# lawfuyang/HobbyRenderer

Measured on AMD Instinct MI355X. Metric: Mrays/s at 1920×1080, 8 spp, 4 bounces; 1/2/4/8 GPU scaling, higher is better.
Workload: dtype f32; 1 GPU; config 2: Cornell-box-class procedural scene (38 triangles, 9 instances, closed room, emissive quad + default sun), 1920x1080, 8 spp (accumulation indices 0..7), 4 bounces; frames_in_flight=2, serial_kernels=False, mode=default

## Files before the change

hobbyrenderer_amd/csrc/pt_capi.cpp:

```cpp
#include <hip/hip_runtime.h>

#include <chrono>
#include <cmath>
#include <cstdio>
#include <cstdlib>
#include <cstring>
#include <mutex>
#include <new>
#include <stdexcept>
#include <limits>
#include <string>
#include <system_error>
#include <thread>
#include <vector>

#include "../../include/hobbyrt_pt.h"
#include "bvh_build.h"
#include "bvh_build_gpu.h"
#include "pt_deform.h"
#include "pt_skin.h"
#include "pt_anim.h"
#include "pt_device.h"
#include "pt_kernels.h"
#include "pt_motion.h"
// ... 188 lines not shown
    if (const char* e = getenv("HRPT_WF_SEGMENT_SHIFT")) c->wf.knobs.segmentShift = (uint32_t)atoi(e);
    if (const char* e = getenv("HRPT_WF_SEGMENT_SIZE")) c->wf.knobs.segmentSize = (uint32_t)atoi(e);
    if (const char* e = getenv("HRPT_WF_BLOCKS_PER_CU")) c->wf.knobs.blocksPerCu = (uint32_t)atoi(e);
    if (const char* e = getenv("HRPT_WF_EXTEND_BLOCKS_PER_CU")) c->wf.knobs.extendBlocksPerCu = (uint32_t)atoi(e);
    if (const char* e = getenv("HRPT_WF_REFILL_MIN")) c->wf.knobs.refillMin = (uint32_t)atoi(e);
    if (const char* e = getenv("HRPT_WF_BVH_WIDTH")) c->wf.knobs.bvhWidth = (uint32_t)atoi(e);
    if (const char* e = getenv("HRPT_BVH_BUILDER")) c->bvhBuilder = (strcmp(e, "ploc") == 0 || strcmp(e, "2") == 0) ? HRPT_BVH_BUILDER_GPU_PLOC : ((strcmp(e, "gpu") == 0 || strcmp(e, "lbvh") == 0 || strcmp(e, "1") == 0) ? HRPT_BVH_BUILDER_GPU_LBVH : ((strcmp(e, "auto") == 0 || strcmp(e, "3") == 0) ? HRPT_BVH_BUILDER_AUTO : HRPT_BVH_BUILDER_HOST_SAH));
    if (const char* e = getenv("HRPT_WF_PAD_LDS")) c->wf.knobs.padLdsBytes = (uint32_t)atoi(e);
    if (const char* e = getenv("HRPT_WF_DRAIN_SEGMENTS")) c->wf.knobs.drainSegments = atoi(e) != 0;
    if (const char* e = getenv("HRPT_WF_SERIAL_SHADOW")) c->wf.knobs.serialShadow = atoi(e) != 0;
    if (const char* e = getenv("HRPT_WF_SHADOW_PATH")) c->wf.knobs.shadowPath = atoi(e);
    if (const char* e = getenv("HRPT_WF_SHADE_SORT")) c->wf.knobs.shadeSort = atoi(e) != 0 ? 1 : 0;
    if (const char* e = getenv("HRPT_WF_SLIM_SHADOW")) c->wf.knobs.noSlimShadow = atoi(e) == 0;
    if (const char* e = getenv("HRPT_WF_FUSED_PRIMARY")) c->wf.knobs.noFusedPrimary = atoi(e) == 0;
    if (const char* e = getenv("HRPT_WF_FUSED_BOUNCE0")) c->wf.knobs.noFusedBounce0 = atoi(e) == 0;
    if (const char* e = getenv("HRPT_WF_SHADE_LDS_TABLES")) c->wf.knobs.noShadeLdsTables = atoi(e) == 0;
    if (const char* e = getenv("HRPT_WF_NODE_LOOP_MIN")) c->wf.knobs.nodeLoopMin = (uint32_t)atoi(e);
    if (const char* e = getenv("HRPT_BLOOM_FUSED_TAIL")) { const int v = atoi(e); c->bloomTailTexels = v == 1 ? 8192u : (v > 0 ? (uint32_t)v : 0u); }
    *out = c;
    return HRPT_OK;
}

void hrpt_destroy(HrptContext* c)
{
    if (!c) return;
    (void)hipSetDevice(c->device);
    if (c->stream) (void)hipStreamSynchronize(c->stream);
    free_scene(c);
    for (AnimDeviceCopy& a : c->animations) free_animation_copy(a);
    wavefront_release(c->wf);
// ... 1873 lines not shown
```

hobbyrenderer_amd/csrc/pt_device.h:

```cpp
#pragma once

#include <hip/hip_runtime.h>
#include <stdint.h>

#include "../../include/hobbyrt_pt.h"
#include "../../include/hobbyrt/detmath.h"
#include "../../include/hobbyrt/srgb_table.h"

#define HRT_DEV __device__ __forceinline__

#if defined(HRPT_PHASE_PROFILE) && defined(HRPT_PHASE_TU)
extern __device__ unsigned long long g_phaseCounters[128];
#define HRT_PHASE(k)                                                                                                      \
    do {                                                                                                                  \
        const unsigned long long m_ = __ballot(true);                                                                     \
        if ((threadIdx.x & 63u) == (unsigned)(__ffsll((long long)m_) - 1)) {                                              \
            atomicAdd(&g_phaseCounters[2 * (k)], 1ull); atomicAdd(&g_phaseCounters[2 * (k) + 1], (unsigned long long)__popcll(m_)); \
        }                                                                                                                 \
    } while (0)
#else
#define HRT_PHASE(k) do { } while (0)
#endif
enum {
    PH_EXT_ITER = 0, PH_EXT_REFILL, PH_EXT_NODE, PH_EXT_LEAF, PH_EXT_TRI, PH_EXT_FINISH, PH_EXT_CANDIDATE,
    PH_ANY_ITER = 8, PH_ANY_REFILL, PH_ANY_NODE, PH_ANY_LEAF, PH_ANY_TRI, PH_ANY_FINISH,
    PH_SHADE_ITER = 16, PH_SHADE_HIT, PH_SHADE_ATTR, PH_SHADE_TEX, PH_SHADE_TRANS, PH_SHADE_NEE, PH_SHADE_LOBE_BEGIN, PH_SHADE_DIFFUSE, PH_SHADE_SPEC,
    PH_SHADE_SKY, PH_SHADE_WRITE, PH_SHADE_SORT,
    PH_SHADOW_ENTRY = 32, PH_SHADOW_SAMPLE, PH_SHADOW_QUERY, PH_SHADOW_CONTRIB, PH_SHADOW_RAYS_ITEM,
    PH_COUNT = 40
};

namespace hrt {

struct f2 { float x, y; };
struct f3 { float x, y, z; };
struct f4 { float x, y, z, w; };

HRT_DEV f3 mk3(float x, float y, float z) { f3 r; r.x = x; r.y = y; r.z = z; return r; }
HRT_DEV f3 mk3(const float* p) { return mk3(p[0], p[1], p[2]); }
HRT_DEV f3 operator+(f3 a, f3 b) { return mk3(a.x + b.x, a.y + b.y, a.z + b.z); }
HRT_DEV f3 operator-(f3 a, f3 b) { return mk3(a.x - b.x, a.y - b.y, a.z - b.z); }
HRT_DEV f3 operator*(f3 a, f3 b) { return mk3(a.x * b.x, a.y * b.y, a.z * b.z); }
HRT_DEV f3 operator*(f3 a, float s) { return mk3(a.x * s, a.y * s, a.z * s); }
HRT_DEV f3 operator/(f3 a, float s) { return mk3(a.x / s, a.y / s, a.z / s); }
// ... 306 lines not shown
                    best.t = take ? t : best.t; best.u = take ? u : best.u; best.v = take ? v : best.v;
                    best.inst = take ? inst : best.inst; best.prim = take ? prim : best.prim; best.tri = take ? first + i : best.tri;
                    best.opaque = take ? (__float_as_uint(c.w) & 1u) : best.opaque;
                    best.valid = best.valid || take;
                    tlim = take ? t : tlim;
                }
            }
            if (sp == 0) break;
            cur = stack.pop(--sp);
        }
    }
    return best;
}

template <class BVH, class STACK>
HRT_DEV bool any_opaque(const BVH& bvh, int32_t rootLeaf, uint32_t nodeCount, const Ray& r, STACK& stack, bool& sawNonOpaque, uint32_t nodeLoopMin = 0)
{
    sawNonOpaque = false;
    if (!(r.d.x == r.d.x && r.d.y == r.d.y && r.d.z == r.d.z)) return false;
    RayShear sh = make_shear(r.d);
    f3 inv = traversal_rcp(r.d), noi = slab_origin_term(r.o, inv);
    int sp = 0; int32_t cur;
    if (nodeCount == 0) { if (rootLeaf == 0) return false; cur = rootLeaf; }
    else cur = 0;
    for (;;) {
        while (cur >= 0) {
            cur = inner_step(bvh, cur, noi, inv, r.tmin, r.tmax, stack, sp);
            if ((uint32_t)__popcll(__ballot(cur >= 0)) < nodeLoopMin) break;
        }
        if (cur == kTraversalDone) break;
        if (cur < 0) {
            uint32_t enc = (uint32_t)(~cur);
            uint32_t first = enc >> 2, count = (enc & 3u) + 1u;
            for (uint32_t i = 0; i < count; ++i) {
                float4 a, b, c; bvh.tri(first + i, a, b, c);
                float t, u, v;
                if (tri_test(mk3(a.x, a.y, a.z), mk3(b.x, b.y, b.z), mk3(c.x, c.y, c.z), r, sh, t, u, v)) {
                    if (__float_as_uint(c.w) & 1u) return true;
                    sawNonOpaque = true;
                }
            }
            if (sp == 0) break;
            cur = stack.pop(--sp);
        }
    }
    return false;
}

constexpr int32_t kExitBlas = 0x7FFFFFFE;
struct GlobalBvhTl : GlobalBvh4 {
    static constexpr bool kTwoLevel = true;
    const GpuInstance* instances;
};
struct TlCull { f3 inv, noi, noiF; int32_t inst; };
HRT_DEV void tl_world(TlCull& c, const Ray& r)
{
    c.inv = traversal_rcp(r.d); c.noi = slab_origin_term(r.o, c.inv); c.noiF = c.noi; c.inst = -1;
}
HRT_DEV void tl_enter(TlCull& c, const GpuInstance& I, int32_t inst, const Ray& r)
// ... 733 lines not shown
```

hobbyrenderer_amd/csrc/pt_path.h:

```cpp
#pragma once

#include "pt_device.h"

namespace hrt {

struct PathState {
    Ray ray;
    uint32_t rng;
    f3 throughput, radiance;
    bool inVolume; float interiorIOR; f3 sigmaA, sigmaS;
};

struct SurfaceCarry {
    f3 N, V, worldPos, baseColor, F0; float Fr, roughness, metallic, ior;
    uint32_t rngBeforeLights;
    uint32_t material;
};

HRT_DEV void init_path(PathState& ps, const HrptPathTracerConstants& cb, uint32_t px, uint32_t py)
{
    float u = (((float)px + 0.5f) + cb.m_Jitter[0]) * cb.m_View.m_ViewportSizeInv[0];
    float v = (((float)py + 0.5f) + cb.m_Jitter[1]) * cb.m_View.m_ViewportSizeInv[1];
    float cx = u * 2.0f + -1.0f, cy = v * -2.0f + 1.0f;
    const float* M = cb.m_View.m_MatClipToWorldNoOffset;
// ... 283 lines not shown
    }
    if (overflow) {
        float4 la, lb, lc; bvh.tri(lastTri, la, lb, lc);
        HitKey lower; lower.have = true; lower.t = lastT; lower.inst = __float_as_uint(la.w); lower.prim = __float_as_uint(lb.w);
        for (;;) {
            Hit h = closest_any(bvh, s.rootLeaf, s.nodeCount, ray, lower, stack);
            if (!h.valid) break;
            if (h.opaque) return 0.0f;
            if (shadow_candidate(s, ray, h.t, h.tri, h.u, h.v, st)) return 0.0f;
            lower.t = h.t; lower.inst = h.inst; lower.prim = h.prim;
        }
    }
    return shadow_finish(ray, st);
}
template <int K, class BVH, class STACK, class CAND>
HRT_DEV float shadow_query_buffered(const SceneView& s, const BVH& bvh, f3 worldPos, f3 L, float maxDist, STACK& stack, CAND& cand, uint32_t nodeLoopMin = 0)
{
    Ray ray = shadow_ray(worldPos, L, maxDist);
    if (!(ray.d.x == ray.d.x && ray.d.y == ray.d.y && ray.d.z == ray.d.z)) return 1.0f;
    RayShear sh = make_shear(ray.d);
    f3 inv = traversal_rcp(ray.d), noi = slab_origin_term(ray.o, inv);
    int sp = 0, count = 0; bool overflow = false;
    int32_t cur;
    if (s.nodeCount == 0) { if (s.rootLeaf == 0) return 1.0f; cur = s.rootLeaf; } else cur = 0;
    for (;;) {
        while (cur >= 0) {
            cur = inner_step(bvh, cur, noi, inv, ray.tmin, ray.tmax, stack, sp);
            if ((uint32_t)__popcll(__ballot(cur >= 0)) < nodeLoopMin) break;
        }
        if (cur == kTraversalDone) break;
        if (cur >= 0) continue;
        uint32_t enc = (uint32_t)(~cur);
        uint32_t first = enc >> 2, n = (enc & 3u) + 1u;
        for (uint32_t i = 0; i < n; ++i) {
            float4 a, b, c; bvh.tri(first + i, a, b, c);
            float t, u, v;
            if (!tri_test(mk3(a.x, a.y, a.z), mk3(b.x, b.y, b.z), mk3(c.x, c.y, c.z), ray, sh, t, u, v)) continue;
            if (__float_as_uint(c.w) & 1u) return 0.0f;
            candidate_insert<K>(bvh, cand, count, overflow, t, first + i, __float_as_uint(a.w), __float_as_uint(b.w));
        }
        if (sp == 0) break;
        cur = stack.pop(--sp);
    }
    return shadow_resolve_candidates(s, bvh, ray, sh, count, overflow, cand, stack);
}

template <bool DIRONLY>
HRT_DEV bool nee_draw(const HrptGPULight& l, f3 N, f3 worldPos, f3 sunDirection, uint32_t& rng, float& ux, float& uy)
{
    if (DIRONLY || l.m_Type == HRPT_LIGHT_DIRECTIONAL) {
        if (dot(N, sunDirection) <= 0.0f) return false;
    } else if (!DIRONLY && (l.m_Type == HRPT_LIGHT_POINT || l.m_Type == HRPT_LIGHT_SPOT)) {
        if (l.m_Intensity <= 0.0f) return false;
// ... 228 lines not shown
```

hobbyrenderer_amd/csrc/pt_wavefront.hip:

```cpp
#define HRPT_PHASE_TU 1
#include "pt_wavefront.h"

#include <mutex>
#include <type_traits>
#include <unordered_map>
#include <vector>

#include "bvh_build.h"
#include "pt_gbuffer.h"
#include "pt_motion.h"
#include "pt_path.h"

#ifdef HRPT_PHASE_PROFILE
__device__ unsigned long long g_phaseCounters[128];
#endif
#ifdef HRPT_SKY_DEBUG
__device__ float g_skyDebug[2048 * 16];
#endif

namespace hrt {

namespace {

constexpr uint32_t kMaxSppPerBatch = 64;
// ... 1013 lines not shown
                if (!valid) a.b.shVis[id] = kVisNoRay;
            }
            const unsigned long long m = __ballot(valid);
            if (valid) {
                const uint32_t o = segBase * a.maxLights + outCount + prefix_rank(m);
                a.b.sqO[o] = make_float4(ray.o.x, ray.o.y, ray.o.z, ray.tmin);
                a.b.sqD[o] = make_float4(ray.d.x, ray.d.y, ray.d.z, ray.tmax);
                a.b.sqId[o] = id;
            }
            outCount += (uint32_t)__popcll(m);
        }
        if (lane == 0) a.b.sqCnt[seg] = outCount;
    }
}

template <bool LDS_BVH, int DEPTH, int W, bool DIRONLY, int MODE, int TL = 0>
__global__ __launch_bounds__(kBlock) __attribute__((amdgpu_waves_per_eu(MODE == 2 && TL == 0 ? 4 : ((MODE == 1 || TL != 0) ? 3 : 1)))) void wf_shadow(WfArgs a, HrptPathTracerConstants cb, int bounce)
{
    static_assert(!TL || (!LDS_BVH && W == 4 && (MODE == kShadowOpaque || MODE == kShadowSlim)), "two-level structure: opaque any-hit query over the global tree");
    static_assert(W != kQuantisedTree || (!LDS_BVH && !TL), "quantised nodes: flat tree in global memory");
    constexpr bool NONOPAQUE = MODE == kShadowBuffered || MODE == kShadowResolve;
    constexpr bool SLIM = MODE == kShadowSlim;
    constexpr int kLdsMax = MODE == kShadowResolve ? kExtendLdsStack : kShadowLdsStack;
    extern __shared__ __attribute__((aligned(128))) char smem[];
    LdsStack<DEPTH, kLdsMax> stack; LdsBvh<W> lbvh;
    constexpr size_t candBytes = MODE == kShadowBuffered ? (size_t)kShadowCandidates * 2 * kBlock * 4 : 0;
    setup_lds<LDS_BVH, DEPTH, W>(smem, a.scene, stack, lbvh, candBytes);
    if (DEPTH > kLdsMax) { stack.spill = a.spill[1] + blockIdx.x * kBlock + threadIdx.x; stack.spillStride = gridDim.x * kBlock; }
    LdsCandidates cand; cand.base = reinterpret_cast<int32_t*>(smem + (size_t)LdsStack<DEPTH, kLdsMax>::kRows * kBlock * 4) + threadIdx.x;
    LdsCandidates3 cand3; cand3.base = cand.base;
    typename GlobalBvhOf<(TL ? kTwoLevelTree : W)>::type gbvh = GlobalBvhOf<(TL ? kTwoLevelTree : W)>::make(a.scene);
    const SceneView& s = a.scene;
    const f3 sunDir = mk3(cb.m_SunDirection[0], cb.m_SunDirection[1], cb.m_SunDirection[2]);
    const float sunIntensity = s.lights[0].m_Intensity;

    const uint32_t wavesPerBlock = kBlock / 64, lane = lane_id();
    const uint32_t gw = uniform(blockIdx.x * wavesPerBlock + (threadIdx.x >> 6)), totalWaves = gridDim.x * wavesPerBlock;
    unsigned int nRays = 0, nSamples = 0, nRadiance = 0, nSkipped16 = 0;
    auto process = [&](uint32_t e) {
                HRT_PHASE(PH_SHADOW_ENTRY);
                if (SLIM) {
                    const float4 h0 = a.b.sh0[e], h1 = a.b.sh1[e];
                    const uint32_t slot = __float_as_uint(h0.w);
                    const float4 rd = a.b.rayD[a.shadowParity][slot];
                    const f3 origin = mk3(h0.x, h0.y, h0.z), N = mk3(h1.x, h1.y, h1.z);
                    uint32_t rng = __float_as_uint(rd.w);
                    const float ux = hrt_rng_next(&rng), uy = hrt_rng_next(&rng);
                    ++nSamples;
                    HrptGPULight l = load_light(s, 0u);
                    f3 L; float maxDist;
                    if (!nee_direction<true>(l, N, origin, sunDir, cb.m_CosSunAngularRadius, ux, uy, L, maxDist)) return;
                    float shadow;
                    if (LDS_BVH) shadow = shadow_query<true>(s, lbvh, origin, L, maxDist, stack);
// ... 40 lines not shown
                    if (MODE == kShadowResolve || j) ls = a.b.shL[(size_t)e * a.maxLights + j];
                    HrptGPULight l = load_light(s, __float_as_uint(ls.z));
                    f3 L; float maxDist;
                    if (!nee_direction<DIRONLY>(l, N, origin, sunDir, cb.m_CosSunAngularRadius, ls.x, ls.y, L, maxDist)) continue;
                    float shadow;
                    HRT_PHASE(PH_SHADOW_QUERY);
                    if (MODE == kShadowResolve) {
                        if (vis == kVisClear) shadow = 1.0f;
                        else {
                            Ray sr = shadow_ray(origin, L, maxDist);
                            GlobalCandidates gc; gc.base = a.b.sqCand + (size_t)(e * a.maxLights + j) * kShadowCandidates;
                            const int cnt = (int)((vis >> 8) & 0xFFu); const bool ovf = (vis >> 16) & 1u;
                            if (LDS_BVH) shadow = shadow_resolve_candidates(s, lbvh, sr, make_shear(sr.d), cnt, ovf, gc, stack);
                            else shadow = shadow_resolve_candidates(s, gbvh, sr, make_shear(sr.d), cnt, ovf, gc, stack);
                        }
                    } else if (MODE == kShadowBuffered) {
                        if (LDS_BVH) shadow = shadow_query_buffered<kShadowCandidates>(s, lbvh, origin, L, maxDist, stack, cand);
                        else shadow = shadow_query_buffered<kShadowCandidates>(s, gbvh, origin, L, maxDist, stack, cand);
                    } else {
                        if (LDS_BVH) shadow = shadow_query<true>(s, lbvh, origin, L, maxDist, stack);
                        else if constexpr (TL == 2) shadow = shadow_query_two_level_buffered<kTwoLevelCandidates>(s, gbvh, shadow_ray(origin, L, maxDist), stack, cand3);
                    else shadow = shadow_query<true>(s, gbvh, origin, L, maxDist, stack);
                    }
                    ++nRays;
                    if (shadow != 0.0f) {
                        HRT_PHASE(PH_SHADOW_CONTRIB);
                        float4 h2 = a.b.sh2[e], h3 = a.b.sh3[e];
                        f3 dif, spec;
                        nee_contribution<DIRONLY>(s, l, nee_lighting(N, mk3(h2.x, h2.y, h2.z), mk3(h3.x, h3.y, h3.z), h1.w, h2.w, h3.w), origin, sunDir,
                                                  sunIntensity, L, dif, spec);
                        totalDiffuse = totalDiffuse + dif * shadow;
                        if (bounce == 0) totalSpecular = totalSpecular + spec * shadow;
                    }
                }
                f3 dsum = totalDiffuse + (bounce == 0 ? totalSpecular : mk3(0.0f, 0.0f, 0.0f));
                if (dsum.x != 0.0f || dsum.y != 0.0f || dsum.z != 0.0f) {
                    f3 term = T * dsum;
                    float4 r = a.b.radiance[smp];
                    r.x = r.x + term.x; r.y = r.y + term.y; r.z = r.z + term.z;
                    a.b.radiance[smp] = r;
                    ++nRadiance;
                }
    };
    if (NONOPAQUE) {
        uint32_t seg = gw, cnt = 0, segBase = 0, next = 0; bool haveSeg = false;
        auto open_segment = [&]() {
            haveSeg = false; cnt = 0; next = 0;
            for (; seg < a.numSegments; seg += totalWaves) {
                cnt = uniform(a.b.shadowCnt[seg]);
                if (cnt) { segBase = seg * a.segSize; haveSeg = true; break; }
            }
        };
        open_segment();
        while (haveSeg) {
            uint32_t e = 0xFFFFFFFFu, filled = 0;
            while (filled < 64u && haveSeg) {
                uint32_t take = cnt - next < 64u - filled ? cnt - next : 64u - filled;
                if (lane >= filled && lane < filled + take) e = segBase + next + (lane - filled);
                next += take; filled += take;
// ... 4 lines not shown
    } else {
        for (uint32_t seg = gw; seg < a.numSegments; seg += totalWaves) {
            const uint32_t cnt = uniform(a.b.shadowCnt[seg]), segBase = seg * a.segSize;
            for (uint32_t base = 0; base < cnt; base += 64) {
                uint32_t i = base + lane;
                if (i < cnt) process(segBase + i);
            }
        }
    }
    block_count_add(&a.counters->closestRays, 1, nRays);
    __syncthreads();
    block_count_add(&a.counters->closestRays, 4, nSamples);
    __syncthreads();
    block_count_add(&a.counters->closestRays, 6, nRadiance);
    if (SLIM && a.primary) { __syncthreads(); block_count_add(&a.counters->closestRays, 7, nSkipped16); }
}

__global__ __launch_bounds__(kBlock) void wf_resolve(WfArgs a, float4* __restrict__ accumulation, float4* __restrict__ output, uint32_t firstIndex)
{
    uint32_t p = blockIdx.x * blockDim.x + threadIdx.x;
    uint32_t stride = gridDim.x * blockDim.x;
    for (; p < a.pixelsPadded; p += stride) {
        uint32_t tile = p >> 6, within = p & 63u;
        uint32_t tcol, trow; tile_position(a, tile, tcol, trow);
        uint32_t px = a.rect.column_x(tcol) + (within & 7u), py = a.rect.y0 + trow * 8u + (within >> 3);
        if (px >= a.rect.x1 || py >= a.rect.y1) continue;
        size_t idx = (size_t)py * a.imageWidth + px;
        float4 acc = make_float4(0.0f, 0.0f, 0.0f, 0.0f);
        for (uint32_t k = 0; k < a.spp; ++k) {
            float4 r = a.b.radiance[(size_t)k * a.pixelsPadded + p];
// ... 115 lines not shown

void launch_extend(const Variant& v, uint32_t cus, dim3 g, hipStream_t st, const WfArgs& a, uint32_t parity, bool anyHit = false)
{
    dispatch_variant(v, [&](auto L, auto D, auto W, auto TL) {
        constexpr bool l = L(); constexpr int d = D(), w = W(), tl = TL();
        auto closest = [&](auto kernel) { launch_rounds(cus, kernel, g, v.ldsBytes, st, a, parity); };
        if constexpr (tl != 0) {
            if (a.primary) closest(wf_extend<false, d, 4, false, tl, true>);
            else closest(wf_extend<false, d, 4, false, tl, false>);
        } else if (anyHit) hipLaunchKernelGGL((wf_extend<l, d, w, true>), g, dim3(kBlock), v.ldsBytes + kCandidateLdsBytes, st, a, parity);
        else if constexpr (w == 2) closest(wf_extend<l, d, w, false>);
        else if (a.primary) { if (a.allOpaque) closest(wf_extend<l, d, w, false, 0, true, true>); else closest(wf_extend<l, d, w, false, 0, true>); }
        else { if (a.allOpaque) closest(wf_extend<l, d, w, false, 0, false, true>); else closest(wf_extend<l, d, w, false>); }
    });
}
void launch_shadow(const Variant& v, dim3 g, hipStream_t st, const WfArgs& a, const HrptPathTracerConstants& cb, int bounce, bool dirOnly, int mode)
{
    dispatch_variant(v, [&](auto L, auto D, auto W, auto TL) {
        constexpr bool l = L(); constexpr int d = D(), w = W(), tl = TL();
        auto launch = [&](auto kernel, size_t extraLds) { hipLaunchKernelGGL(kernel, g, dim3(kBlock), v.ldsBytes + extraLds, st, a, cb, bounce); };
        if constexpr (tl != 0) {
            const size_t cand = tl == 2 ? (size_t)kTwoLevelCandidates * 3 * kBlock * 4 : 0;
            if (mode == kShadowSlim) launch(wf_shadow<false, d, 4, true, kShadowSlim, tl>, cand);
            else if (dirOnly) launch(wf_shadow<false, d, 4, true, kShadowOpaque, tl>, cand);
            else launch(wf_shadow<false, d, 4, false, kShadowOpaque, tl>, cand);
        } else if (mode == kShadowResolve) launch(wf_shadow<l, d, w, false, kShadowResolve>, 0);
        else if (mode == kShadowBuffered) launch(wf_shadow<l, d, w, false, kShadowBuffered>, kCandidateLdsBytes);
        else if (mode == kShadowSlim) launch(wf_shadow<l, d, w, true, kShadowSlim>, 0);
        else if (dirOnly) launch(wf_shadow<l, d, w, true, kShadowOpaque>, 0);
        else launch(wf_shadow<l, d, w, false, kShadowOpaque>, 0);
    });
}
void launch_wf_trace_rays(const Variant& v, uint32_t cus, dim3 g, hipStream_t st, const WfTraceArgs& a, bool shadow)
{
    dispatch_variant(v, [&](auto L, auto D, auto W, auto TL) {
        constexpr bool l = L(), tl = TL() != 0; constexpr int d = D(), w = W();
        if constexpr (w != 2) {
            if (shadow) launch_rounds(cus, wf_trace_rays<l, d, w, true, tl>, g, v.ldsBytes + (tl ? 0 : kCandidateLdsBytes), st, a);
            else launch_rounds(cus, wf_trace_rays<l, d, w, false, tl>, g, v.ldsBytes, st, a);
        }
    });
// ... 254 lines not shown
            if (!st.auxStream && hipStreamCreateWithFlags(&st.auxStream, hipStreamNonBlocking) != hipSuccess) { st.auxStream = nullptr; overlap = false; }
            while (overlap && st.forkEvents.size() < (size_t)maxBounces) {
                hipEvent_t f, j;
                if (hipEventCreateWithFlags(&f, hipEventDisableTiming) != hipSuccess) { overlap = false; break; }
                if (hipEventCreateWithFlags(&j, hipEventDisableTiming) != hipSuccess) { (void)hipEventDestroy(f); overlap = false; break; }
                st.forkEvents.push_back(f); st.joinEvents.push_back(j);
            }
        }
        auto shadow_stage = [&](hipStream_t sst, int bounce) {
            a.shadowParity = (uint32_t)bounce & 1u;
            if (plan.shadowMode == kShadowResolve) {
                if (traits.directionalLightsOnly) hipLaunchKernelGGL((wf_shadow_rays<true>), grid, dim3(kBlock), 0, sst, a, cb);
                else hipLaunchKernelGGL((wf_shadow_rays<false>), grid, dim3(kBlock), 0, sst, a, cb);
                launch_extend(plan.vA, cus, grid, sst, a, 0u, true);
            }
            launch_shadow(plan.vS, grid, sst, a, cb, bounce, traits.directionalLightsOnly, plan.shadowMode);
        };
        bool pendingJoin = false;
        for (int bounce = 0; bounce < maxBounces; ++bounce) {
            const uint32_t parity = (uint32_t)bounce & 1u;
            const bool timed = st.profile && st.eventsUsed + 8 <= 4096;
            a.primary = (fusedPrimary && bounce == 0) ? 1u : 0u;
            const bool fusedBounce0 = plan.fusedBounce0 && bounce == 0;
            if (timed && !fusedBounce0) timing_mark(st, stream, 0, true);
            if (!fusedBounce0) launch_extend(plan.vE, cus, dim3(batch.gridExtend), stream, a, parity);
            if (timed) { if (!fusedBounce0) timing_mark(st, stream, 0, false); timing_mark(st, stream, 1, true); }
            if (pendingJoin) { if ((e = hipStreamWaitEvent(stream, st.joinEvents[(size_t)bounce - 1], 0)) != hipSuccess) { error = "hipStreamWaitEvent(join)"; return e; } pendingJoin = false; }
            const int last = bounce + 1 == maxBounces ? 1 : 0;
            const size_t sortLds = (size_t)(kBlock / 64) * ((size_t)5 * a.segSize);
            if (fusedBounce0) {
                if (plan.vE.depth <= 16) hipLaunchKernelGGL((wf_bounce0<16>), grid, dim3(kBlock), plan.bounce0LdsBytes, stream, a, cb, last);
// ... 106 lines not shown
```

hobbyrenderer_amd/csrc/pt_wavefront_plan.h:

```cpp
#pragma once

#include <stddef.h>
#include <stdint.h>

namespace hrt {

struct SceneTraits {
    bool hasMedium = false;
    bool hasStochasticAlpha = false;
    bool hasTextures = false;
    bool hasTransmissiveOrBlend = false;
    bool directionalLightsOnly = true;
    bool hasNonOpaque = false;
    uint32_t bvhMaxDepth = 0;
    uint32_t bvh4MaxDepth = 0;
    bool quantisedNodes = false;
    uint32_t twoLevelStackNeed = 0;
};

struct TreeCounts {
    uint32_t nodeCount = 0, node4Count = 0, triCount = 0;
    bool hasNodesQ = false, hasInstances = false;
    uint32_t instanceCount = 0, materialCount = 0;
};
// ... 3 lines not shown
    uint32_t extendBlocksPerCu = 0;
    uint32_t refillMin = 0;
    uint32_t segmentShift = 0;
    uint32_t segmentSize = 0;
    bool drainSegments = false;
    bool serialShadow = false;
    uint32_t padLdsBytes = 0;
    uint32_t bvhWidth = 0;
    uint32_t nodeLoopMin = ~0u;
    bool noFusedPrimary = false;
    bool noSlimShadow = false;
    int shadeSort = -1;
    bool noFusedBounce0 = false;
    bool noShadeLdsTables = false;
    int shadowPath = 0;
};

constexpr uint32_t kMaxSegment = 1024;
constexpr uint32_t kBlock = 256;
constexpr uint32_t kMaxLights = 8;
constexpr size_t kLdsBudget = 64 * 1024;
constexpr int kExtendLdsStack = 16, kShadowLdsStack = 32;
constexpr uint32_t kMaxStackNeed = 128;
constexpr int kShadowCandidates = 8;
constexpr int kTwoLevelCandidates = 4;
constexpr size_t kCandidateLdsBytes = (size_t)kShadowCandidates * 2 * kBlock * 4;
#ifndef HRPT_LDS_NODE4_STRIDE
#define HRPT_LDS_NODE4_STRIDE 128
#endif
constexpr uint32_t kLdsNode4Stride = HRPT_LDS_NODE4_STRIDE;
// ... 3 lines not shown
constexpr size_t kShadeRingBytes = (size_t)(kBlock / 64) * kShadeRing * kShadeRingFields * 4;
constexpr uint32_t kShadeBlocksPerCu = 4;
constexpr size_t kCuLdsBytes = 160 * 1024, kShadeLdsMargin = 1024;
constexpr size_t kShadeLdsPerBlock = kCuLdsBytes / kShadeBlocksPerCu - kShadeLdsMargin;
constexpr size_t kTriAttrBytes = 80, kInstShadeBytes = 48, kMaterialBytes = 180;
constexpr size_t shade_table_bytes(uint32_t triCount, uint32_t instanceCount, uint32_t materialCount)
{
    const size_t b = (size_t)triCount * kTriAttrBytes + (size_t)instanceCount * kInstShadeBytes + (size_t)materialCount * kMaterialBytes;
    return (b + 15) & ~(size_t)15;
}
constexpr uint32_t kBounce0Ring = 32;
constexpr size_t kBounce0RingBytes = (size_t)(kBlock / 64) * kBounce0Ring * kShadeRingFields * 4;
static_assert(kBounce0RingBytes % 128 == 0, "the tree copy behind ring and tables starts 128-byte aligned");
constexpr size_t bounce0_shade_bytes(size_t tableBytes) { return kBounce0RingBytes + ((tableBytes + 127) & ~(size_t)127); }
enum : int { kShadowOpaque = 0, kShadowBuffered = 1, kShadowResolve = 2, kShadowSlim = 3 };

struct Variant { bool lds = false; int depth = 0, width = 0; size_t ldsBytes = 0; bool twoLevel = false; bool twoLevelCandidates = false; bool quantised = false; };

inline uint32_t stack_entries4(uint32_t depth4) { return 3 * depth4 + 3; }
inline uint32_t stack_need4(const SceneTraits& traits) { return traits.twoLevelStackNeed ? traits.twoLevelStackNeed : stack_entries4(traits.bvh4MaxDepth); }

inline Variant pick_variant(const SceneTraits& traits, const TreeCounts& tree, int width, size_t extraBytes, int ldsStackMax, size_t padBytes)
{
    Variant v; v.width = width;
    uint32_t need = traits.twoLevelStackNeed;
    if (need) { v.width = 4; v.twoLevel = true; v.twoLevelCandidates = traits.hasNonOpaque; }
    else {
        if (v.width == 4 && stack_entries4(traits.bvh4MaxDepth) > kMaxStackNeed) v.width = 2;
        need = v.width == 2 ? traits.bvhMaxDepth + 2 : stack_entries4(traits.bvh4MaxDepth);
    }
    v.depth = (v.width == 2 && need <= 8) ? 8 : (need <= 16 ? 16 : (need <= 32 ? 32 : 64));
    const size_t bvhBytes = v.twoLevel ? 0 : (v.width == 2 ? (size_t)tree.nodeCount * 64 : (size_t)tree.node4Count * kLdsNode4Stride) + (size_t)tree.triCount * 48;
    const size_t stackBytes = (size_t)(v.depth > ldsStackMax ? ldsStackMax : v.depth) * kBlock * 4;
    v.lds = bvhBytes > 0 && stackBytes + extraBytes + bvhBytes <= kLdsBudget;
    v.ldsBytes = stackBytes + (v.lds ? bvhBytes : 0) + padBytes;
    v.quantised = v.width == 4 && !v.lds && !v.twoLevel && traits.quantisedNodes && tree.hasNodesQ;
    return v;
}

struct RenderPlan {
    Variant vE, vS, vA;
    int shadowMode = kShadowOpaque;
    bool slim = false;
    bool simpleScene = false;
    bool fusedPrimary = false;
    uint32_t sortShade = 0, nodeLoopMin = 0;
    uint32_t maxLights = 1, cus = 0, blocksPerCu = 0, extendBlocksPerCu = 0;
    uint32_t spillEntries = 0; size_t spillThreads = 0;
    uint32_t pathRecordBytes = 48; uint64_t bytesPerSample = 0;
    bool shadeLdsTables = false;
    size_t shadeTableBytes = 0;
    size_t shadeLdsBytes = 0;
    bool fusedBounce0 = false;
    size_t bounce0LdsBytes = 0;
};
struct BatchPlan { uint32_t segSize, numSegments, grid, gridExtend; };

inline RenderPlan plan_render(const SceneTraits& traits, const TreeCounts& tree, uint32_t lightCount, uint32_t cus, const WavefrontKnobs& k)
// ... 11 lines not shown
    p.vE = pick(forced ? forced : 4, 0, kExtendLdsStack);
    p.vS = pick(forced ? forced : 4, candBytes, kShadowLdsStack);
    if (!forced && p.vS.lds && !traits.hasNonOpaque) p.vS = pick(2, candBytes, kShadowLdsStack);
    const bool manyLights = maxLights > 1;
    const bool unevenRays = manyLights || (traits.hasNonOpaque && traits.hasTransmissiveOrBlend);
    const int selfMode = traits.hasNonOpaque ? kShadowBuffered : kShadowOpaque;
    p.shadowMode = (!p.vS.lds && unevenRays) ? kShadowResolve : selfMode;
    if (k.shadowPath == 1) p.shadowMode = selfMode;
    if (k.shadowPath == 2 && (traits.hasNonOpaque || manyLights)) p.shadowMode = kShadowResolve;
    if (traits.twoLevelStackNeed) p.shadowMode = kShadowOpaque;
    p.vA = pick(forced ? forced : 4, kCandidateLdsBytes, kExtendLdsStack);
    if (p.shadowMode == kShadowResolve) p.vS = pick(forced ? forced : 4, 0, kExtendLdsStack);
    p.simpleScene = !traits.hasTextures && !traits.hasTransmissiveOrBlend && traits.directionalLightsOnly;
    p.slim = p.simpleScene && !manyLights && p.shadowMode == kShadowOpaque && !k.noSlimShadow;
    if (p.slim) p.shadowMode = kShadowSlim;
    p.nodeLoopMin = k.nodeLoopMin != ~0u ? k.nodeLoopMin : (p.vE.lds ? 16u : 24u);
    p.blocksPerCu = k.blocksPerCu ? k.blocksPerCu : ((k.serialShadow && !p.vE.lds) ? 8 : 16);
    p.extendBlocksPerCu = k.extendBlocksPerCu ? k.extendBlocksPerCu : (k.blocksPerCu ? k.blocksPerCu : (p.vE.lds ? 12u : 6u));
    if (p.vE.depth > kExtendLdsStack || p.vS.depth > kShadowLdsStack) {
        const uint32_t worst = traits.twoLevelStackNeed ? traits.twoLevelStackNeed : (p.vE.width == 4 || p.vS.width == 4 ? stack_entries4(traits.bvh4MaxDepth) : traits.bvhMaxDepth + 2);
        p.spillEntries = worst > (uint32_t)kExtendLdsStack ? worst - kExtendLdsStack : 1u;
        p.spillThreads = (size_t)cus * (p.blocksPerCu > p.extendBlocksPerCu ? p.blocksPerCu : p.extendBlocksPerCu) * kBlock;
    }
    p.shadeLdsBytes = kShadeRingBytes;
    if (p.simpleScene && !manyLights && !k.noShadeLdsTables && !tree.hasInstances && !traits.twoLevelStackNeed &&
        tree.triCount && tree.instanceCount && tree.materialCount) {
        const size_t tables = shade_table_bytes(tree.triCount, tree.instanceCount, tree.materialCount);
        if (kShadeRingBytes + tables <= kShadeLdsPerBlock) { p.shadeLdsTables = true; p.shadeTableBytes = tables; p.shadeLdsBytes = kShadeRingBytes + tables; }
    }
    p.fusedPrimary = p.simpleScene && !manyLights && maxLights <= kMaxLights && p.vE.width == 4 && !traits.hasMedium && !traits.hasStochasticAlpha && !k.noFusedPrimary;
// ... 65 lines not shown
```

hobbyrenderer_amd/scenes.py:

```python
import math

import numpy as np

from . import structs as S

f32 = np.float32


def quantize_snorm(v, bits):
    scale = f32((1 << (bits - 1)) - 1)
    rnd = f32(0.5) if v >= 0 else f32(-0.5)
    v = f32(max(-1.0, min(1.0, float(v))))
    return int(f32(v * scale) + rnd)


def quantize_half(v):
    ui = int(np.array(v, f32).view(np.uint32))
    s = (ui >> 16) & 0x8000
    em = ui & 0x7FFFFFFF
    h = (em - (112 << 23) + (1 << 12)) >> 13
    if em < (113 << 23):
        h = 0
    if em >= (143 << 23):
        h = 0x7C00
# ... 143 lines not shown
    mat = b.add_material()
    b.add_instance(mesh, mat)
    return b.finalize(luts)


_ROT_TO = {
    "+y": [[1, 0, 0], [0, 1, 0], [0, 0, 1]],
    "-y": [[-1, 0, 0], [0, -1, 0], [0, 0, 1]],
    "+x": [[0, -1, 0], [1, 0, 0], [0, 0, 1]],
    "-x": [[0, 1, 0], [-1, 0, 0], [0, 0, 1]],
    "+z": [[1, 0, 0], [0, 0, 1], [0, -1, 0]],
    "-z": [[1, 0, 0], [0, 0, -1], [0, 1, 0]],
}


def cornell_scene(luts, extra_lights=False):
    b = SceneBuilder()
    quad = b.add_mesh(*generate_floor_quad())
    cube = b.add_mesh(*generate_default_cube())
    white = b.add_material(m_BaseColor=(0.73, 0.73, 0.73, 1))
    red = b.add_material(m_BaseColor=(0.65, 0.05, 0.05, 1))
    green = b.add_material(m_BaseColor=(0.12, 0.45, 0.15, 1))
    light = b.add_material(m_BaseColor=(0.78, 0.78, 0.78, 1), m_EmissiveFactor=(17, 12, 4, 1))
    zc, zl = -1.5, 5.0
    b.add_instance(quad, white, _mat((2, 1, zl), _ROT_TO["+y"], (0, 0, zc)))
    b.add_instance(quad, white, _mat((2, 1, zl), _ROT_TO["-y"], (0, 2, zc)))
    b.add_instance(quad, red, _mat((2, 1, zl), _ROT_TO["+x"], (-1, 1, zc)))
    b.add_instance(quad, green, _mat((2, 1, zl), _ROT_TO["-x"], (1, 1, zc)))
    b.add_instance(quad, white, _mat((2, 1, 2), _ROT_TO["-z"], (0, 1, 1)))
    b.add_instance(quad, white, _mat((2, 1, 2), _ROT_TO["+z"], (0, 1, -4)))
    c, s = 0.96, 0.28
    b.add_instance(cube, white, _mat((0.6, 0.6, 0.6), [[c, 0, -s], [0, 1, 0], [s, 0, c]], (0.35, 0.3, -0.15)))
    b.add_instance(cube, white, _mat((0.6, 1.2, 0.6), [[c, 0, s], [0, 1, 0], [-s, 0, c]], (-0.35, 0.6, 0.35)))
    b.add_instance(quad, light, _mat((0.5, 1, 0.5), _ROT_TO["-y"], (0, 1.98, 0)))
    if extra_lights:
        b.add_light(S.LIGHT_POINT, position=(0.5, 1.5, -0.5), color=(1.0, 0.9, 0.8), intensity=3.0, radius=0.05, range_=10.0)
        b.add_light(S.LIGHT_SPOT, position=(-0.6, 1.8, -1.0), direction=(0.3, -1.0, 0.4), color=(0.6, 0.7, 1.0), intensity=6.0,
                    radius=0.02, inner=0.3, outer=0.6)
    return b.finalize(luts)


# ... 46 lines not shown
    cb["m_FrameIndex"] = frame_index
    cb["m_MaxBounces"] = max_bounces
    cb["m_Jitter"] = (halton(accumulation_index + 1, 2) - f32(0.5), halton(accumulation_index + 1, 3) - f32(0.5))
    cb["m_SunDirection"] = scene.sun_direction
    half_angle = f32(scene.sun_angular_size_deg) * f32(0.5) * (f32(3.141592654) / f32(180.0))
    cb["m_CosSunAngularRadius"] = f32(math.cos(float(half_angle)))
    return cb


def config_cube(luts, size=256):
    sc = cube_scene(luts)
    view, pos = planar_view(size, size, aspect=1.0)
    return sc, view, pos, dict(spp=1, max_bounces=1)


def config_cornell(luts, width=1920, height=1080, extra_lights=False):
    sc = cornell_scene(luts, extra_lights)
    view, pos = planar_view(width, height, position=(0.0, 1.0, -3.4), fov_y=math.radians(40.0), aspect=16.0 / 9.0)
    return sc, view, pos, dict(spp=8, max_bounces=4)


def quantize_snorm_array(v, bits):
    v = np.clip(np.asarray(v, f32), f32(-1.0), f32(1.0))
    scale = f32((1 << (bits - 1)) - 1)
    rnd = np.where(v >= 0, f32(0.5), f32(-0.5)).astype(f32)
    return (v * scale + rnd).astype(f32).astype(np.int32)


def quantize_half_array(v):
    ui = np.asarray(v, f32).view(np.uint32).astype(np.int64)
    s = (ui >> 16) & 0x8000
    em = ui & 0x7FFFFFFF
# ... 194 lines not shown
```

Measured before the change: 27180 Mrays/s.

## Add per-thread shadow blocker cache and sparse-lane parking ring in shadow stage

Each thread remembers the last one or two BVH leaves that held an opaque occluder. Before a full traversal it tests those leaves and skips the any-hit traversal when one of them still blocks the ray. This targets closed scenes where most sun shadow rays hit the same geometry. For slim mode, sparse waves with few active shadow queries are parked in a per-wave LDS ring and flushed as denser batches to reduce divergence. In exchange it spends extra LDS and registers and adds wasted leaf tests when the cache misses. It is on by default for LDS-tree opaque modes.

```diff
diff --git a/hobbyrenderer_amd/csrc/pt_capi.cpp b/hobbyrenderer_amd/csrc/pt_capi.cpp
--- a/hobbyrenderer_amd/csrc/pt_capi.cpp
+++ b/hobbyrenderer_amd/csrc/pt_capi.cpp
@@ -226,6 +226,7 @@
     if (const char* e = getenv("HRPT_WF_SLIM_SHADOW")) c->wf.knobs.noSlimShadow = atoi(e) == 0;
     if (const char* e = getenv("HRPT_WF_FUSED_PRIMARY")) c->wf.knobs.noFusedPrimary = atoi(e) == 0;
     if (const char* e = getenv("HRPT_WF_FUSED_BOUNCE0")) c->wf.knobs.noFusedBounce0 = atoi(e) == 0;
+    if (const char* e = getenv("HRPT_WF_SHADOW_CACHE")) c->wf.knobs.shadowCache = atoi(e) != 0 ? 1 : 0;
     if (const char* e = getenv("HRPT_WF_SHADE_LDS_TABLES")) c->wf.knobs.noShadeLdsTables = atoi(e) == 0;
     if (const char* e = getenv("HRPT_WF_NODE_LOOP_MIN")) c->wf.knobs.nodeLoopMin = (uint32_t)atoi(e);
     if (const char* e = getenv("HRPT_BLOOM_FUSED_TAIL")) { const int v = atoi(e); c->bloomTailTexels = v == 1 ? 8192u : (v > 0 ? (uint32_t)v : 0u); }
diff --git a/hobbyrenderer_amd/csrc/pt_device.h b/hobbyrenderer_amd/csrc/pt_device.h
--- a/hobbyrenderer_amd/csrc/pt_device.h
+++ b/hobbyrenderer_amd/csrc/pt_device.h
@@ -27,7 +27,8 @@
     PH_SHADE_ITER = 16, PH_SHADE_HIT, PH_SHADE_ATTR, PH_SHADE_TEX, PH_SHADE_TRANS, PH_SHADE_NEE, PH_SHADE_LOBE_BEGIN, PH_SHADE_DIFFUSE, PH_SHADE_SPEC,
     PH_SHADE_SKY, PH_SHADE_WRITE, PH_SHADE_SORT,
     PH_SHADOW_ENTRY = 32, PH_SHADOW_SAMPLE, PH_SHADOW_QUERY, PH_SHADOW_CONTRIB, PH_SHADOW_RAYS_ITEM,
-    PH_COUNT = 40
+    PH_SHADOW_CACHE_TEST, PH_SHADOW_CACHE_HIT, PH_SHADOW_PARK, PH_SHADOW_FLUSH,
+    PH_COUNT = 44
 };
 
 namespace hrt {
@@ -364,7 +365,7 @@
 }
 
 template <class BVH, class STACK>
-HRT_DEV bool any_opaque(const BVH& bvh, int32_t rootLeaf, uint32_t nodeCount, const Ray& r, STACK& stack, bool& sawNonOpaque, uint32_t nodeLoopMin = 0)
+HRT_DEV bool any_opaque(const BVH& bvh, int32_t rootLeaf, uint32_t nodeCount, const Ray& r, STACK& stack, bool& sawNonOpaque, uint32_t nodeLoopMin = 0, uint32_t* blockerLeaf = nullptr)
 {
     sawNonOpaque = false;
     if (!(r.d.x == r.d.x && r.d.y == r.d.y && r.d.z == r.d.z)) return false;
@@ -386,13 +387,25 @@
                 float4 a, b, c; bvh.tri(first + i, a, b, c);
                 float t, u, v;
                 if (tri_test(mk3(a.x, a.y, a.z), mk3(b.x, b.y, b.z), mk3(c.x, c.y, c.z), r, sh, t, u, v)) {
-                    if (__float_as_uint(c.w) & 1u) return true;
+                    if (__float_as_uint(c.w) & 1u) { if (blockerLeaf) *blockerLeaf = enc; return true; }
                     sawNonOpaque = true;
                 }
             }
             if (sp == 0) break;
             cur = stack.pop(--sp);
         }
+    }
+    return false;
+}
+
+template <class BVH>
+HRT_DEV bool leaf_blocks(const BVH& bvh, uint32_t enc, const Ray& r, const RayShear& sh)
+{
+    const uint32_t first = enc >> 2, count = (enc & 3u) + 1u;
+    for (uint32_t i = 0; i < count; ++i) {
+        float4 a, b, c; bvh.tri(first + i, a, b, c);
+        float t, u, v;
+        if ((__float_as_uint(c.w) & 1u) && tri_test(mk3(a.x, a.y, a.z), mk3(b.x, b.y, b.z), mk3(c.x, c.y, c.z), r, sh, t, u, v)) return true;
     }
     return false;
 }
diff --git a/hobbyrenderer_amd/csrc/pt_path.h b/hobbyrenderer_amd/csrc/pt_path.h
--- a/hobbyrenderer_amd/csrc/pt_path.h
+++ b/hobbyrenderer_amd/csrc/pt_path.h
@@ -321,7 +321,7 @@
     return shadow_finish(ray, st);
 }
 template <int K, class BVH, class STACK, class CAND>
-HRT_DEV float shadow_query_buffered(const SceneView& s, const BVH& bvh, f3 worldPos, f3 L, float maxDist, STACK& stack, CAND& cand, uint32_t nodeLoopMin = 0)
+HRT_DEV float shadow_query_buffered(const SceneView& s, const BVH& bvh, f3 worldPos, f3 L, float maxDist, STACK& stack, CAND& cand, uint32_t nodeLoopMin = 0, uint32_t* blockerLeaf = nullptr)
 {
     Ray ray = shadow_ray(worldPos, L, maxDist);
     if (!(ray.d.x == ray.d.x && ray.d.y == ray.d.y && ray.d.z == ray.d.z)) return 1.0f;
@@ -343,7 +343,7 @@
             float4 a, b, c; bvh.tri(first + i, a, b, c);
             float t, u, v;
             if (!tri_test(mk3(a.x, a.y, a.z), mk3(b.x, b.y, b.z), mk3(c.x, c.y, c.z), ray, sh, t, u, v)) continue;
-            if (__float_as_uint(c.w) & 1u) return 0.0f;
+            if (__float_as_uint(c.w) & 1u) { if (blockerLeaf) *blockerLeaf = enc; return 0.0f; }
             candidate_insert<K>(bvh, cand, count, overflow, t, first + i, __float_as_uint(a.w), __float_as_uint(b.w));
         }
         if (sp == 0) break;
diff --git a/hobbyrenderer_amd/csrc/pt_wavefront.hip b/hobbyrenderer_amd/csrc/pt_wavefront.hip
--- a/hobbyrenderer_amd/csrc/pt_wavefront.hip
+++ b/hobbyrenderer_amd/csrc/pt_wavefront.hip
@@ -1051,17 +1051,46 @@
     }
 }
 
-template <bool LDS_BVH, int DEPTH, int W, bool DIRONLY, int MODE, int TL = 0>
-__global__ __launch_bounds__(kBlock) __attribute__((amdgpu_waves_per_eu(MODE == 2 && TL == 0 ? 4 : ((MODE == 1 || TL != 0) ? 3 : 1)))) void wf_shadow(WfArgs a, HrptPathTracerConstants cb, int bounce)
+constexpr uint32_t kNoLeaf = 0xFFFFFFFFu;
+#ifndef HRPT_BC_SECOND_LEAF_MIN
+#define HRPT_BC_SECOND_LEAF_MIN 24
+#endif
+constexpr uint32_t kSecondLeafMin = HRPT_BC_SECOND_LEAF_MIN;
+struct BlockerCache {
+    uint32_t leaf0 = kNoLeaf, leaf1 = kNoLeaf, score = 0;
+    HRT_DEV void learn(uint32_t leaf)
+    {
+        if (leaf != leaf0) { leaf1 = leaf0; leaf0 = leaf; }
+        score = score < 2u ? 2u : score;
+    }
+    template <class BVH> HRT_DEV bool blocks(const BVH& bvh, const Ray& r)
+    {
+        auto finite = [](float x) { return __builtin_fabsf(x) < __builtin_inff(); };
+        if (!score || !(finite(r.o.x) && finite(r.o.y) && finite(r.o.z) && finite(r.d.x) && finite(r.d.y) && finite(r.d.z) && finite(r.tmax))) return false;
+        HRT_PHASE(PH_SHADOW_CACHE_TEST);
+        const RayShear sh = make_shear(r.d);
+        bool hit = leaf_blocks(bvh, leaf0, r, sh);
+        const bool second = !hit && leaf1 != kNoLeaf;
+        const uint32_t nSecond = (uint32_t)__popcll(__ballot(second));
+        if (second && nSecond >= kSecondLeafMin && leaf_blocks(bvh, leaf1, r, sh)) { const uint32_t t = leaf0; leaf0 = leaf1; leaf1 = t; hit = true; }
+        if (hit) HRT_PHASE(PH_SHADOW_CACHE_HIT);
+        score = hit ? 3u : score - 1u;
+        return hit;
+    }
+};
+
+template <bool LDS_BVH, int DEPTH, int W, bool DIRONLY, int MODE, int TL, bool CACHE>
+HRT_DEV void shadow_stage(const WfArgs& a, const HrptPathTracerConstants& cb, int bounce)
 {
     static_assert(!TL || (!LDS_BVH && W == 4 && (MODE == kShadowOpaque || MODE == kShadowSlim)), "two-level structure: opaque any-hit query over the global tree");
     static_assert(W != kQuantisedTree || (!LDS_BVH && !TL), "quantised nodes: flat tree in global memory");
+    static_assert(!CACHE || (!TL && MODE != kShadowResolve), "blocker cache: the modes that traverse a flat tree themselves");
     constexpr bool NONOPAQUE = MODE == kShadowBuffered || MODE == kShadowResolve;
     constexpr bool SLIM = MODE == kShadowSlim;
     constexpr int kLdsMax = MODE == kShadowResolve ? kExtendLdsStack : kShadowLdsStack;
     extern __shared__ __attribute__((aligned(128))) char smem[];
     LdsStack<DEPTH, kLdsMax> stack; LdsBvh<W> lbvh;
-    constexpr size_t candBytes = MODE == kShadowBuffered ? (size_t)kShadowCandidates * 2 * kBlock * 4 : 0;
+    constexpr size_t candBytes = MODE == kShadowBuffered ? (size_t)kShadowCandidates * 2 * kBlock * 4 : ((CACHE && SLIM) ? kShadowRingBytes : 0);
     setup_lds<LDS_BVH, DEPTH, W>(smem, a.scene, stack, lbvh, candBytes);
     if (DEPTH > kLdsMax) { stack.spill = a.spill[1] + blockIdx.x * kBlock + threadIdx.x; stack.spillStride = gridDim.x * kBlock; }
     LdsCandidates cand; cand.base = reinterpret_cast<int32_t*>(smem + (size_t)LdsStack<DEPTH, kLdsMax>::kRows * kBlock * 4) + threadIdx.x;
@@ -1074,6 +1103,90 @@
     const uint32_t wavesPerBlock = kBlock / 64, lane = lane_id();
     const uint32_t gw = uniform(blockIdx.x * wavesPerBlock + (threadIdx.x >> 6)), totalWaves = gridDim.x * wavesPerBlock;
     unsigned int nRays = 0, nSamples = 0, nRadiance = 0, nSkipped16 = 0;
+    [[maybe_unused]] BlockerCache bc;
+    [[maybe_unused]] auto with_tree = [&](auto&& f) { if constexpr (LDS_BVH) return f(lbvh); else return f(gbvh); };
+    if constexpr (CACHE && SLIM) {
+        constexpr uint32_t kDense = 16, kNoEntry = 0xFFFFFFFFu;
+        uint32_t* const ring = reinterpret_cast<uint32_t*>(smem + (size_t)LdsStack<DEPTH, kLdsMax>::kRows * kBlock * 4) + (size_t)uniform(threadIdx.x >> 6) * kShadowRing;
+        uint32_t head = 0, pending = 0;
+        uint32_t seg = gw, cnt = 0, segBase = 0, next = 0; bool haveSeg = false;
+        auto open_segment = [&]() {
+            haveSeg = false; cnt = 0; next = 0;
+            for (; seg < a.numSegments; seg += totalWaves) {
+                cnt = uniform(a.b.shadowCnt[seg]);
+                if (cnt) { segBase = seg * a.segSize; haveSeg = true; break; }
+            }
+        };
+        open_segment();
+        const HrptGPULight l = load_light(s, 0u);
+        for (;;) {
+            const bool drain = pending >= 64u || !haveSeg;
+            if (drain && pending == 0u) break;
+            uint32_t e = kNoEntry;
+            if (drain) {
+                const uint32_t n = pending < 64u ? pending : 64u;
+                if (lane < n) e = ring[(head + lane) & (kShadowRing - 1u)];
+                head = (head + n) & (kShadowRing - 1u); pending -= n;
+                __builtin_amdgcn_fence(__ATOMIC_SEQ_CST, "wavefront");
+            } else {
+                if (next + lane < cnt) e = segBase + next + lane;
+                next += 64u;
+                if (next >= cnt) { seg += totalWaves; open_segment(); }
+            }
+            bool need = false;
+            float4 h1 = make_float4(0.0f, 0.0f, 0.0f, 0.0f), rd = h1; uint32_t slot = 0;
+            f3 origin = mk3(0.0f, 0.0f, 0.0f), N = origin, L = origin; float maxDist = 0.0f;
+            if (e != kNoEntry) {
+                HRT_PHASE(PH_SHADOW_ENTRY);
+                const float4 h0 = a.b.sh0[e]; h1 = a.b.sh1[e];
+                slot = __float_as_uint(h0.w);
+                rd = a.b.rayD[a.shadowParity][slot];
+                origin = mk3(h0.x, h0.y, h0.z); N = mk3(h1.x, h1.y, h1.z);
+                uint32_t rng = __float_as_uint(rd.w);
+                const float ux = hrt_rng_next(&rng), uy = hrt_rng_next(&rng);
+                if (!drain) ++nSamples;
+                need = nee_direction<true>(l, N, origin, sunDir, cb.m_CosSunAngularRadius, ux, uy, L, maxDist);
+            }
+            const Ray ray = shadow_ray(origin, L, maxDist);
+            if (!drain) {
+                if (need && with_tree([&](const auto& bvh) { return bc.blocks(bvh, ray); })) { need = false; ++nRays; }
+                const unsigned long long m = __ballot(need);
+                const uint32_t n = (uint32_t)__popcll(m);
+                if (n && n < kDense) {
+                    if (need) { HRT_PHASE(PH_SHADOW_PARK); ring[(head + pending + prefix_rank(m)) & (kShadowRing - 1u)] = e; }
+                    need = false; pending += n;
+                    __builtin_amdgcn_fence(__ATOMIC_SEQ_CST, "wavefront");
+                }
+            }
+            if (need) {
+                if (drain) HRT_PHASE(PH_SHADOW_FLUSH); else HRT_PHASE(PH_SHADOW_QUERY);
+                uint32_t leaf = kNoLeaf; bool sawNonOpaque;
+                const bool blocked = with_tree([&](const auto& bvh) { return any_opaque(bvh, s.rootLeaf, s.nodeCount, ray, stack, sawNonOpaque, 0u, &leaf); });
+                ++nRays;
+                if (blocked) bc.learn(leaf);
+                else {
+                    const float shadow = 1.0f;
+                    const float4 th = a.primary ? make_float4(1.0f, 1.0f, 1.0f, __uint_as_float(slot)) : a.b.thr[a.shadowParity][slot];
+                    if (a.primary) ++nSkipped16;
+                    const HrptMaterialConstants& mat = s.materials[__float_as_uint(h1.w)];
+                    f3 dif, spec;
+                    nee_contribution<true>(s, l, nee_lighting(N, mk3(-rd.x, -rd.y, -rd.z), mk3(mat.m_BaseColor), hrt_max(mat.m_RoughnessMetallic[0], 0.04f),
+                                                              mat.m_RoughnessMetallic[1], mat.m_IOR), origin, sunDir, sunIntensity, L, dif, spec);
+                    f3 totalDiffuse = mk3(0.0f, 0.0f, 0.0f) + dif * shadow, totalSpecular = mk3(0.0f, 0.0f, 0.0f);
+                    if (bounce == 0) totalSpecular = totalSpecular + spec * shadow;
+                    const f3 dsum = totalDiffuse + (bounce == 0 ? totalSpecular : mk3(0.0f, 0.0f, 0.0f));
+                    if (dsum.x != 0.0f || dsum.y != 0.0f || dsum.z != 0.0f) {
+                        const f3 term = mk3(th.x, th.y, th.z) * dsum;
+                        const uint32_t smp = __float_as_uint(th.w);
+                        float4 r = a.b.radiance[smp];
+                        r.x = r.x + term.x; r.y = r.y + term.y; r.z = r.z + term.z;
+                        a.b.radiance[smp] = r;
+                        ++nRadiance;
+                    }
+                }
+            }
+        }
+    }
     auto process = [&](uint32_t e) {
                 HRT_PHASE(PH_SHADOW_ENTRY);
                 if (SLIM) {
@@ -1144,6 +1257,15 @@
                             if (LDS_BVH) shadow = shadow_resolve_candidates(s, lbvh, sr, make_shear(sr.d), cnt, ovf, gc, stack);
                             else shadow = shadow_resolve_candidates(s, gbvh, sr, make_shear(sr.d), cnt, ovf, gc, stack);
                         }
+                    } else if constexpr (CACHE) {
+                        const Ray ray = shadow_ray(origin, L, maxDist);
+                        if (with_tree([&](const auto& bvh) { return bc.blocks(bvh, ray); })) shadow = 0.0f;
+                        else {
+                            uint32_t leaf = kNoLeaf;
+                            if constexpr (MODE == kShadowBuffered) shadow = with_tree([&](const auto& bvh) { return shadow_query_buffered<kShadowCandidates>(s, bvh, origin, L, maxDist, stack, cand, 0u, &leaf); });
+                            else { bool sawNonOpaque; shadow = with_tree([&](const auto& bvh) { return any_opaque(bvh, s.rootLeaf, s.nodeCount, ray, stack, sawNonOpaque, 0u, &leaf); }) ? 0.0f : 1.0f; }
+                            if (leaf != kNoLeaf) bc.learn(leaf);
+                        }
                     } else if (MODE == kShadowBuffered) {
                         if (LDS_BVH) shadow = shadow_query_buffered<kShadowCandidates>(s, lbvh, origin, L, maxDist, stack, cand);
                         else shadow = shadow_query_buffered<kShadowCandidates>(s, gbvh, origin, L, maxDist, stack, cand);
@@ -1172,7 +1294,8 @@
                     ++nRadiance;
                 }
     };
-    if (NONOPAQUE) {
+    if constexpr (CACHE && SLIM) { (void)process; }
+    else if (NONOPAQUE) {
         uint32_t seg = gw, cnt = 0, segBase = 0, next = 0; bool haveSeg = false;
         auto open_segment = [&]() {
             haveSeg = false; cnt = 0; next = 0;
@@ -1207,6 +1330,16 @@
     __syncthreads();
     block_count_add(&a.counters->closestRays, 6, nRadiance);
     if (SLIM && a.primary) { __syncthreads(); block_count_add(&a.counters->closestRays, 7, nSkipped16); }
+}
+template <bool LDS_BVH, int DEPTH, int W, bool DIRONLY, int MODE, int TL = 0>
+__global__ __launch_bounds__(kBlock) __attribute__((amdgpu_waves_per_eu(MODE == 2 && TL == 0 ? 4 : ((MODE == 1 || TL != 0) ? 3 : 1)))) void wf_shadow(WfArgs a, HrptPathTracerConstants cb, int bounce)
+{
+    shadow_stage<LDS_BVH, DEPTH, W, DIRONLY, MODE, TL, false>(a, cb, bounce);
+}
+template <bool LDS_BVH, int DEPTH, int W, bool DIRONLY, int MODE>
+__global__ __launch_bounds__(kBlock) __attribute__((amdgpu_waves_per_eu(MODE == 1 ? 3 : 1))) void wf_shadow_bc(WfArgs a, HrptPathTracerConstants cb, int bounce)
+{
+    shadow_stage<LDS_BVH, DEPTH, W, DIRONLY, MODE, 0, true>(a, cb, bounce);
 }
 
 __global__ __launch_bounds__(kBlock) void wf_resolve(WfArgs a, float4* __restrict__ accumulation, float4* __restrict__ output, uint32_t firstIndex)
@@ -1352,7 +1485,7 @@
         else { if (a.allOpaque) closest(wf_extend<l, d, w, false, 0, false, true>); else closest(wf_extend<l, d, w, false>); }
     });
 }
-void launch_shadow(const Variant& v, dim3 g, hipStream_t st, const WfArgs& a, const HrptPathTracerConstants& cb, int bounce, bool dirOnly, int mode)
+void launch_shadow(const Variant& v, dim3 g, hipStream_t st, const WfArgs& a, const HrptPathTracerConstants& cb, int bounce, bool dirOnly, int mode, bool cache)
 {
     dispatch_variant(v, [&](auto L, auto D, auto W, auto TL) {
         constexpr bool l = L(); constexpr int d = D(), w = W(), tl = TL();
@@ -1363,6 +1496,12 @@
             else if (dirOnly) launch(wf_shadow<false, d, 4, true, kShadowOpaque, tl>, cand);
             else launch(wf_shadow<false, d, 4, false, kShadowOpaque, tl>, cand);
         } else if (mode == kShadowResolve) launch(wf_shadow<l, d, w, false, kShadowResolve>, 0);
+        else if (cache) {
+            if (mode == kShadowBuffered) launch(wf_shadow_bc<l, d, w, false, kShadowBuffered>, kCandidateLdsBytes);
+            else if (mode == kShadowSlim) launch(wf_shadow_bc<l, d, w, true, kShadowSlim>, kShadowRingBytes);
+            else if (dirOnly) launch(wf_shadow_bc<l, d, w, true, kShadowOpaque>, 0);
+            else launch(wf_shadow_bc<l, d, w, false, kShadowOpaque>, 0);
+        }
         else if (mode == kShadowBuffered) launch(wf_shadow<l, d, w, false, kShadowBuffered>, kCandidateLdsBytes);
         else if (mode == kShadowSlim) launch(wf_shadow<l, d, w, true, kShadowSlim>, 0);
         else if (dirOnly) launch(wf_shadow<l, d, w, true, kShadowOpaque>, 0);
@@ -1647,7 +1786,7 @@
                 else hipLaunchKernelGGL((wf_shadow_rays<false>), grid, dim3(kBlock), 0, sst, a, cb);
                 launch_extend(plan.vA, cus, grid, sst, a, 0u, true);
             }
-            launch_shadow(plan.vS, grid, sst, a, cb, bounce, traits.directionalLightsOnly, plan.shadowMode);
+            launch_shadow(plan.vS, grid, sst, a, cb, bounce, traits.directionalLightsOnly, plan.shadowMode, plan.shadowCache);
         };
         bool pendingJoin = false;
         for (int bounce = 0; bounce < maxBounces; ++bounce) {
diff --git a/hobbyrenderer_amd/csrc/pt_wavefront_plan.h b/hobbyrenderer_amd/csrc/pt_wavefront_plan.h
--- a/hobbyrenderer_amd/csrc/pt_wavefront_plan.h
+++ b/hobbyrenderer_amd/csrc/pt_wavefront_plan.h
@@ -41,6 +41,7 @@
     bool noFusedBounce0 = false;
     bool noShadeLdsTables = false;
     int shadowPath = 0;
+    int shadowCache = -1;
 };
 
 constexpr uint32_t kMaxSegment = 1024;
@@ -74,6 +75,9 @@
 static_assert(kBounce0RingBytes % 128 == 0, "the tree copy behind ring and tables starts 128-byte aligned");
 constexpr size_t bounce0_shade_bytes(size_t tableBytes) { return kBounce0RingBytes + ((tableBytes + 127) & ~(size_t)127); }
 enum : int { kShadowOpaque = 0, kShadowBuffered = 1, kShadowResolve = 2, kShadowSlim = 3 };
+constexpr uint32_t kShadowRing = 128;
+constexpr size_t kShadowRingBytes = (size_t)(kBlock / 64) * kShadowRing * 4;
+static_assert(kShadowRingBytes % 128 == 0, "the tree copy behind the ring starts 128-byte aligned");
 
 struct Variant { bool lds = false; int depth = 0, width = 0; size_t ldsBytes = 0; bool twoLevel = false; bool twoLevelCandidates = false; bool quantised = false; };
 
@@ -102,6 +106,7 @@
     Variant vE, vS, vA;
     int shadowMode = kShadowOpaque;
     bool slim = false;
+    bool shadowCache = false;
     bool simpleScene = false;
     bool fusedPrimary = false;
     uint32_t sortShade = 0, nodeLoopMin = 0;
@@ -143,6 +148,12 @@
     p.simpleScene = !traits.hasTextures && !traits.hasTransmissiveOrBlend && traits.directionalLightsOnly;
     p.slim = p.simpleScene && !manyLights && p.shadowMode == kShadowOpaque && !k.noSlimShadow;
     if (p.slim) p.shadowMode = kShadowSlim;
+    {
+        const bool opaqueMode = p.shadowMode == kShadowSlim || p.shadowMode == kShadowOpaque;
+        const bool hasKernel = !traits.twoLevelStackNeed && (opaqueMode || p.shadowMode == kShadowBuffered) &&
+                               (p.shadowMode != kShadowSlim || p.vS.ldsBytes + kShadowRingBytes <= kLdsBudget);
+        p.shadowCache = hasKernel && (k.shadowCache < 0 ? (p.vS.lds && opaqueMode) : k.shadowCache != 0);
+    }
     p.nodeLoopMin = k.nodeLoopMin != ~0u ? k.nodeLoopMin : (p.vE.lds ? 16u : 24u);
     p.blocksPerCu = k.blocksPerCu ? k.blocksPerCu : ((k.serialShadow && !p.vE.lds) ? 8 : 16);
     p.extendBlocksPerCu = k.extendBlocksPerCu ? k.extendBlocksPerCu : (k.blocksPerCu ? k.blocksPerCu : (p.vE.lds ? 12u : 6u));
diff --git a/hobbyrenderer_amd/scenes.py b/hobbyrenderer_amd/scenes.py
--- a/hobbyrenderer_amd/scenes.py
+++ b/hobbyrenderer_amd/scenes.py
@@ -181,7 +181,7 @@
 }
 
 
-def cornell_scene(luts, extra_lights=False):
+def cornell_scene(luts, extra_lights=False, ceiling=True):
     b = SceneBuilder()
     quad = b.add_mesh(*generate_floor_quad())
     cube = b.add_mesh(*generate_default_cube())
@@ -191,7 +191,8 @@
     light = b.add_material(m_BaseColor=(0.78, 0.78, 0.78, 1), m_EmissiveFactor=(17, 12, 4, 1))
     zc, zl = -1.5, 5.0
     b.add_instance(quad, white, _mat((2, 1, zl), _ROT_TO["+y"], (0, 0, zc)))
-    b.add_instance(quad, white, _mat((2, 1, zl), _ROT_TO["-y"], (0, 2, zc)))
+    if ceiling:
+        b.add_instance(quad, white, _mat((2, 1, zl), _ROT_TO["-y"], (0, 2, zc)))
     b.add_instance(quad, red, _mat((2, 1, zl), _ROT_TO["+x"], (-1, 1, zc)))
     b.add_instance(quad, green, _mat((2, 1, zl), _ROT_TO["-x"], (1, 1, zc)))
     b.add_instance(quad, white, _mat((2, 1, 2), _ROT_TO["-z"], (0, 1, 1)))
@@ -268,8 +269,8 @@
     return sc, view, pos, dict(spp=1, max_bounces=1)
 
 
-def config_cornell(luts, width=1920, height=1080, extra_lights=False):
-    sc = cornell_scene(luts, extra_lights)
+def config_cornell(luts, width=1920, height=1080, extra_lights=False, ceiling=True):
+    sc = cornell_scene(luts, extra_lights, ceiling)
     view, pos = planar_view(width, height, position=(0.0, 1.0, -3.4), fov_y=math.radians(40.0), aspect=16.0 / 9.0)
     return sc, view, pos, dict(spp=8, max_bounces=4)
 
```

Result: no change. 27370 Mrays/s (median of 3 runs) (+0.7%).
